# ayushpradhan-dev/robust-speech-analysis-framework

Measured on AMD Instinct MI355X. Metric: audio-seconds processed/sec (extract+CNN-LSTM fwd), higher is better.
Workload: dtype f32

## Files before the change

robust_speech_analysis_framework_amd/csrc/gemm_f16x3.h:

```cpp
#pragma once
#include "gemm_f32.h"

namespace rsaf {

struct GemmH3Params {
    const uint16_t* A;
    int64_t a_plane, lda, sA;
    const float* a_scale;
    int a_scale_zs, a_scale_ms;
    const uint16_t* B;
    int64_t b_plane, ldb;
    const float* b_scale;
    float* C;
    int64_t ldc, sC;
    uint16_t* Cp;
    int64_t c_plane, ldcp, sCp;
    const float* c_scale;
    int c_scale_zs, c_scale_ms;
    unsigned* amax_out;
    int amax_zs;
    const int* amax_row_slot;
    int amax_col_min;
    const float* bias;
    const float* R;
    int64_t ldr, sR;
    int M, N, K, nz;
    const int64_t* ztab;
    const int* row_tab;
    int act;
    float alpha;
    int group_m;
    int a_panel, b_panel, cp_panel;
    int nz2;
    int64_t sA2, sB2, sC2, sBias2;
    int b_panel_rows;
    int a_panel_rows, a_tap_panels, a_tap_inv;
};

int launch_gemm_f16x3(const GemmH3Params& p, hipStream_t stream, const char* tag);

int launch_f16x2_row_scales(const float* src, int64_t rows, int K, int64_t ld, float* scale, float* norm2, unsigned* stat_max,
                            hipStream_t stream);
int launch_split_f16x2(const float* src, int64_t rows, int K, int64_t ld, const float* scale, int scale_stride, uint16_t* planes,
                       int64_t plane_stride, int panels, hipStream_t stream);
int launch_scale_from_bound(const unsigned* amax_bits, int64_t n, const float* factor_dev, float factor_host, const float* add_dev,
                            float* scale, hipStream_t stream);

__host__ __device__ inline float f16x2_scale_for_bound(float bound) {
    union { float f; unsigned u; } v;
    v.f = bound;
    const int e = (int)((v.u >> 23) & 0xff);
    if (e == 0) return 1.0f;
    int se = 127 + 14 - (e - 127);
    se = se < 1 ? 1 : (se > 254 ? 254 : se);
    v.u = (unsigned)se << 23;
    return v.f;
}
__host__ __device__ inline float pow2_inverse(float s) {
    union { float f; unsigned u; } v;
    v.f = s;
    v.u = 0x7F000000u - v.u;
    return v.f;
}

#if defined(__HIPCC__)
typedef float gelu_f32x2 __attribute__((ext_vector_type(2)));
__device__ __forceinline__ gelu_f32x2 gelu_pair(gelu_f32x2 x) {
    const gelu_f32x2 a = x * 0.70710678118654752440f;
    gelu_f32x2 t;
    t.x = __builtin_fabsf(a.x); t.y = __builtin_fabsf(a.y);
    const gelu_f32x2 s = a * a;
    auto K = [](float v) { return gelu_f32x2{v, v}; };
    gelu_f32x2 r = __builtin_elementwise_fma(K(-2.4937484340625815e-05f), t, K(5.528365727514029e-04f));
    const gelu_f32x2 u = __builtin_elementwise_fma(K(-5.603376310318708e-03f), t, K(3.4992024302482605e-02f));
    r = __builtin_elementwise_fma(r, s, u);
    r = __builtin_elementwise_fma(r, t, K(-1.540479063987732e-01f));
    r = __builtin_elementwise_fma(r, t, K(-9.158901572227478e-01f));
    r = __builtin_elementwise_fma(r, t, K(-1.8570011854171753e-01f));
    r = __builtin_elementwise_fma(r, t, t * -1.4426950216293335f);
    gelu_f32x2 e;
    e.x = __builtin_amdgcn_exp2f(r.x); e.y = __builtin_amdgcn_exp2f(r.y);
    gelu_f32x2 far = K(1.0f) - e;
    far.x = __builtin_copysignf(far.x, a.x); far.y = __builtin_copysignf(far.y, a.y);
    gelu_f32x2 q = __builtin_elementwise_fma(K(-5.96761703e-4f), s, K(4.99119423e-3f));
    q = __builtin_elementwise_fma(q, s, K(-2.67681349e-2f));
    q = __builtin_elementwise_fma(q, s, K(1.12819925e-1f));
    q = __builtin_elementwise_fma(q, s, K(-3.76125336e-1f));
    q = __builtin_elementwise_fma(q, s, K(1.28379166e-1f));
    const gelu_f32x2 near = __builtin_elementwise_fma(q, a, a);
    gelu_f32x2 er;
    er.x = t.x > 0.927734375f ? far.x : near.x;
    er.y = t.y > 0.927734375f ? far.y : near.y;
    const gelu_f32x2 hx = x * 0.5f;
    return __builtin_elementwise_fma(hx, er, hx);
}
#endif

}
```

robust_speech_analysis_framework_amd/csrc/gemm_f16x3.hip:

```cpp
#include <algorithm>

#include "gemm_f16x3.h"

namespace rsaf {

using f32x16 = __attribute__((ext_vector_type(16))) float;
using f16x8 = __attribute__((ext_vector_type(8))) _Float16;
typedef __attribute__((address_space(3))) void* lds_ptr3;
typedef const __attribute__((address_space(1))) void* glb_ptr3;

__device__ __forceinline__ unsigned short f16_bits(_Float16 h) { return __builtin_bit_cast(unsigned short, h); }

__device__ __forceinline__ void split2(float xs, unsigned short& h, unsigned short& l) {
    const _Float16 hh = (_Float16)xs;
    const _Float16 ll = (_Float16)(xs - (float)hh);
    h = f16_bits(hh);
    l = f16_bits(ll);
}

template <int TM_, int TN_, int WM_, int WN_, int NST_, int WGS_>
struct H3Cfg {
    static constexpr int TM = TM_, TN = TN_, WM = WM_, WN = WN_, NST = NST_, WGS = WGS_;
    static constexpr int BM = 32 * TM * WM, BN = 32 * TN * WN, BK = 16, NPL = 2;
    static constexpr int THREADS = 64 * WM * WN;
    static constexpr int A_PLANE = BM * BK, B_PLANE = BN * BK;
    static constexpr int STAGE = NPL * (A_PLANE + B_PLANE);
    static constexpr int A_INSTR = BM / 32, B_INSTR = BN / 32;
    static constexpr int PATCH_BYTES = WM * WN * 32 * 36 * 4;
    static constexpr int TAB_BYTES = 2 * (BM + BN) * 4 + 2 * BM * 4;
    static constexpr bool PATCH_IN_STAGE2 = BM > 256;
    static_assert(!PATCH_IN_STAGE2 || STAGE * 2 >= PATCH_BYTES, "stage 2 must hold the epilogue patches");
    static constexpr int LDS_BYTES = NST * STAGE * 2 + (PATCH_IN_STAGE2 ? 0 : PATCH_BYTES) + TAB_BYTES;
};

#if defined(__HIP_DEVICE_COMPILE__)
#define H3_OPAQUE(SP, LB) asm volatile("" : "+s"(SP), "+v"(LB))
#else
#define H3_OPAQUE(SP, LB) (void)0
#endif
#define H3_ADDR(UNIFORM_BASE, LANE_BYTES)                                                                      \
    ({                                                                                                         \
        const char* sp_ = reinterpret_cast<const char*>(UNIFORM_BASE);                                         \
        unsigned lb_ = (LANE_BYTES);                                                                           \
        H3_OPAQUE(sp_, lb_);                                                                                   \
        (glb_ptr3)(sp_ + lb_);                                                                                 \
    })

template <class CFG, int ACT, bool OUT_F32, bool OUT_PLANES, bool HAS_R, bool ROWTAB = false>
__global__ __launch_bounds__(CFG::THREADS, CFG::WGS * CFG::THREADS / 256) void gemm_f16x3_kernel(const GemmH3Params p) {
    extern __shared__ __attribute__((aligned(1024))) unsigned short smem3[];
    constexpr int BM = CFG::BM, BN = CFG::BN, BK = CFG::BK, STAGE = CFG::STAGE, NST = CFG::NST, NPL = CFG::NPL;
    constexpr int TM = CFG::TM, TN = CFG::TN, NW = CFG::WM * CFG::WN;
    constexpr int A_PLANE = CFG::A_PLANE, B_PLANE = CFG::B_PLANE;

    const int tid = threadIdx.x, lane = tid & 63, wave = __builtin_amdgcn_readfirstlane(tid >> 6), l31 = lane & 31, h = lane >> 5;
    const int tiles_n = (p.N + BN - 1) / BN, tiles_m = (p.M + BM - 1) / BM;
    const int nwg = tiles_n * tiles_m;
    const int64_t total_tiles = (int64_t)nwg * p.nz;
    const int wm0 = (wave / CFG::WN) * (32 * TM), wn0 = (wave % CFG::WN) * (32 * TN);

    struct Tile { int m0, n0, Mz; int64_t z, z1, z2, coff; };
    auto tile_at = [&](int64_t t) {
        Tile T;
        T.z = t / nwg;
        const int orig = (int)(t - T.z * nwg);
        T.z1 = p.nz2 > 1 ? T.z / p.nz2 : T.z;
        T.z2 = p.nz2 > 1 ? T.z % p.nz2 : 0;
        T.Mz = p.ztab ? (int)p.ztab[2 * T.z1] : p.M;
        T.coff = p.ztab ? p.ztab[2 * T.z1 + 1] : -1;
        const int xcd = orig & 7, q8 = nwg >> 3, r8 = nwg & 7;
        const int wg = (xcd < r8 ? xcd * (q8 + 1) : r8 * (q8 + 1) + (xcd - r8) * q8) + (orig >> 3);
        const int GROUP_M = p.group_m;
        const int per_group = GROUP_M * tiles_n;
        const int grp = wg / per_group;
        const int first_m = grp * GROUP_M;
        const int gsz = (tiles_m - first_m) < GROUP_M ? (tiles_m - first_m) : GROUP_M;
        const int in_grp = wg - grp * per_group;
        T.m0 = (first_m + in_grp % gsz) * BM;
        T.n0 = (in_grp / gsz) * BN;
        return T;
    };
    auto next_valid = [&](int64_t t, Tile& T) {
        for (; t < total_tiles; t += gridDim.x) {
            T = tile_at(t);
            if (T.m0 < T.Mz) return t;
        }
        return (int64_t)-1;
    };

    constexpr int NI = CFG::A_INSTR + CFG::B_INSTR;
    constexpr int IPW = (NI + NW - 1) / NW;
    const unsigned short* sbase[IPW];
    unsigned voff[IPW];
    int64_t pstride[IPW], kstride[IPW];
    int ldsoff[IPW];
    bool live[IPW];
#pragma unroll
    for (int i = 0; i < IPW; ++i) {
        const int j = wave + NW * i;
        live[i] = j < NI;
        const bool isA = j < CFG::A_INSTR;
        const int jj = isA ? j : j - CFG::A_INSTR;
        pstride[i] = isA ? p.a_plane : p.b_plane;
        kstride[i] = isA ? (p.a_panel ? (int64_t)(p.a_panel_rows > 0 ? p.a_panel_rows : p.M) * 16 : 16) : (p.b_panel ? (int64_t)(p.b_panel_rows > 0 ? p.b_panel_rows : p.N) * 16 : 16);
        ldsoff[i] = isA ? jj * 512 : NPL * A_PLANE + jj * 512;
    }
    auto set_tile = [&](const Tile& T) {
#pragma unroll
        for (int i = 0; i < IPW; ++i) {
            const int j = wave + NW * i;
            const bool isA = j < CFG::A_INSTR;
            const int jj = isA ? j : j - CFG::A_INSTR;
            const int row = 32 * jj + (lane >> 1);
            const int dch = (lane & 1) ^ ((row >> 3) & 1);
            if (isA) {
                const int rr = (T.m0 + row < T.Mz) ? row : T.Mz - 1 - T.m0;
                const int64_t rs = p.a_panel ? 16 : p.lda;
                sbase[i] = p.A + T.z1 * p.sA + T.z2 * p.sA2 + (int64_t)T.m0 * rs;
                voff[i] = 2u * ((unsigned)rr * (unsigned)rs + 8u * dch);
            } else {
                const int rr = (T.n0 + row < p.N) ? row : p.N - 1 - T.n0;
                const int64_t rs = p.b_panel ? 16 : p.ldb;
                sbase[i] = p.B + T.z2 * p.sB2 + (int64_t)T.n0 * rs;
                voff[i] = 2u * ((unsigned)rr * (unsigned)rs + 8u * dch);
            }
        }
    };
    const int nk = p.K / BK;
    auto koff = [&](int i, int KT) -> int64_t {
        if (p.a_tap_panels > 0 && (wave + NW * i) < CFG::A_INSTR) {
            const int tap = (int)(((unsigned)KT * (unsigned)p.a_tap_inv) >> 16);
            return (int64_t)(KT - tap * p.a_tap_panels) * kstride[i] + (int64_t)tap * 16;
        }
        return (int64_t)KT * kstride[i];
    };

#define H3_DMA(KT, ST)                                                                                          \
    do {                                                                                                        \
        _Pragma("unroll") for (int i = 0; i < IPW; ++i) {                                                       \
            if (live[i]) {                                                                                      \
                const bool isA_ = (wave + NW * i) < CFG::A_INSTR;                                               \
                _Pragma("unroll") for (int pl = 0; pl < NPL; ++pl)                                              \
                    __builtin_amdgcn_global_load_lds(H3_ADDR(sbase[i] + (pl * pstride[i] + koff(i, (KT))), voff[i]), \
                        (lds_ptr3)(smem3 + (ST) * STAGE + ldsoff[i] + pl * (isA_ ? A_PLANE : B_PLANE)), 16, 0, 0); \
            }                                                                                                   \
        }                                                                                                       \
    } while (0)

    static_assert(NST == 3 && TM % 2 == 0, "the staggered loop needs three stages and an even number of m-tiles");
    const int grpB = wave >= NW / 2 ? 1 : 0;
    constexpr int NDMA = NPL * IPW;
    constexpr int HM = TM / 2;
    constexpr int PATCH_LD = 36;
    float* patch = reinterpret_cast<float*>(smem3 + (CFG::PATCH_IN_STAGE2 ? 2 : NST) * STAGE) + wave * (32 * PATCH_LD);

    constexpr int TPT = (BM + BN + CFG::THREADS - 1) / CFG::THREADS;
    float* tab0 = reinterpret_cast<float*>(smem3 + NST * STAGE) + (CFG::PATCH_IN_STAGE2 ? 0 : NW * (32 * PATCH_LD));
    float* tab1 = tab0 + (BM + BN);
    int* tab_slot = reinterpret_cast<int*>(tab1 + (BM + BN));
    int* tab_dest = tab_slot + BM;
    float e0[TPT], e1[TPT];
    int e_slot[TPT], e_dest[TPT];
    auto load_epi = [&](const Tile& T) {
#pragma unroll
        for (int u = 0; u < TPT; ++u) {
            const int i = tid + u * CFG::THREADS;
            e0[u] = 1.0f; e1[u] = 0.0f;
            if (i < BM) {
                const int row = T.m0 + i < T.Mz ? T.m0 + i : T.Mz - 1;
                if (ROWTAB) {
                    const int2 rt = reinterpret_cast<const int2*>(p.row_tab)[row];
                    e_slot[u] = rt.x; e_dest[u] = rt.y;
                    e0[u] = p.a_scale[rt.x];
                    e1[u] = (OUT_PLANES && p.Cp) ? p.c_scale[rt.x] : 1.0f;
                } else {
                    e0[u] = p.a_scale[T.z1 * p.a_scale_zs + (int64_t)row * p.a_scale_ms];
                    e1[u] = (OUT_PLANES && p.Cp) ? p.c_scale[T.z1 * p.c_scale_zs + (int64_t)row * p.c_scale_ms] : 1.0f;
                }
            } else if (i < BM + BN) {
                const int col = T.n0 + i - BM;
                e0[u] = col < p.N ? p.b_scale[T.z2 * p.sBias2 + col] : 1.0f;
                e1[u] = (p.bias && col < p.N) ? p.bias[T.z2 * p.sBias2 + col] : 0.0f;
            }
        }
    };
    Tile cur;
    int64_t t_cur = next_valid(blockIdx.x, cur);
    if (t_cur < 0) return;
    load_epi(cur);
    set_tile(cur);
    H3_DMA(0, 0);
    if (nk > 1) H3_DMA(1, 1);

    while (true) {
    f32x16 acc[TM][TN];
#pragma unroll
    for (int i = 0; i < TM; ++i)
#pragma unroll
        for (int j = 0; j < TN; ++j)
#pragma unroll
            for (int e = 0; e < 16; ++e) acc[i][j][e] = 0.0f;

    asm volatile("s_waitcnt vmcnt(0)" ::: "memory");
    if (grpB) __builtin_amdgcn_s_barrier();
    int st = 0;
    for (int kt = 0; kt < nk; ++kt) {
        if (!grpB) asm volatile("s_waitcnt vmcnt(0)" ::: "memory");
        __builtin_amdgcn_s_barrier();
        asm volatile("" ::: "memory");
        const int rkt = kt + 1 + grpB;
        const bool refill = rkt < nk && (grpB || kt >= 1);
        const int rst = (st + 1 + grpB) % NST;
        const unsigned short* img = smem3 + st * STAGE;
        f16x8 bf[TN][NPL];
#pragma unroll
        for (int nt = 0; nt < TN; ++nt) {
            const int row = wn0 + nt * 32 + l31;
            const int off = row * BK + ((h ^ ((row >> 3) & 1)) << 3);
#pragma unroll
            for (int pl = 0; pl < NPL; ++pl) bf[nt][pl] = *reinterpret_cast<const f16x8*>(&img[NPL * A_PLANE + pl * B_PLANE + off]);
        }
        if (refill) {
#pragma unroll
            for (int d = 0; d < NDMA; ++d) {
                const int i = d / NPL, pl = d % NPL;
                if (live[i]) {
                    const bool isA_ = (wave + NW * i) < CFG::A_INSTR;
                    __builtin_amdgcn_sched_barrier(0);
                    __builtin_amdgcn_global_load_lds(H3_ADDR(sbase[i] + (pl * pstride[i] + koff(i, rkt)), voff[i]),
                        (lds_ptr3)(smem3 + rst * STAGE + ldsoff[i] + pl * (isA_ ? A_PLANE : B_PLANE)), 16, 0, 0);
                    __builtin_amdgcn_sched_barrier(0);
                }
            }
        }
        f16x8 afp[NPL];
#pragma unroll
        for (int mt = 0; mt < TM; ++mt) {
            f16x8 af[NPL];
            if (mt == HM) {
#pragma unroll
                for (int pl = 0; pl < NPL; ++pl) af[pl] = afp[pl];
            } else {
                const int row = wm0 + mt * 32 + l31;
                const int off = row * BK + ((h ^ ((row >> 3) & 1)) << 3);
#pragma unroll
                for (int pl = 0; pl < NPL; ++pl) af[pl] = *reinterpret_cast<const f16x8*>(&img[pl * A_PLANE + off]);
            }
            if (mt == HM - 1) {
                const int row = wm0 + HM * 32 + l31;
                const int off = row * BK + ((h ^ ((row >> 3) & 1)) << 3);
#pragma unroll
                for (int pl = 0; pl < NPL; ++pl) afp[pl] = *reinterpret_cast<const f16x8*>(&img[pl * A_PLANE + off]);
            }
#pragma unroll
            for (int nt = 0; nt < TN; ++nt) {
                f32x16 c = acc[mt][nt];
                c = __builtin_amdgcn_mfma_f32_32x32x16_f16(af[1], bf[nt][0], c, 0, 0, 0);
                c = __builtin_amdgcn_mfma_f32_32x32x16_f16(af[0], bf[nt][1], c, 0, 0, 0);
                c = __builtin_amdgcn_mfma_f32_32x32x16_f16(af[0], bf[nt][0], c, 0, 0, 0);
                acc[mt][nt] = c;
            }
            if (mt == HM - 1) {
                if (grpB) {
                    if (!refill) asm volatile("s_waitcnt vmcnt(0)" ::: "memory");
                    else if (live[IPW - 1]) asm volatile("s_waitcnt vmcnt(%0)" ::"n"(NPL * IPW) : "memory");
                    else asm volatile("s_waitcnt vmcnt(%0)" ::"n"(NPL * (IPW - 1) > 0 ? NPL * (IPW - 1) : 0) : "memory");
                }
                __builtin_amdgcn_s_barrier();
                asm volatile("" ::: "memory");
            }
        }
        st = st == NST - 1 ? 0 : st + 1;
    }
    if (!grpB) __builtin_amdgcn_s_barrier();

    const Tile done = cur;
    constexpr int CW = (OUT_PLANES && !OUT_F32) ? 8 : 4, LPR = 32 / CW, RPI = 64 / LPR, NQ = 32 / RPI;
    const int lr = lane / LPR, c4 = CW * (lane % LPR);
    float4 r4[4];
    auto load_r = [&](int mt, int nt) {
        const int tn = done.n0 + wn0 + nt * 32, tm = done.m0 + wm0 + mt * 32;
        const float* Rt = p.R + done.z * p.sR + (int64_t)tm * p.ldr + tn + c4;
#pragma unroll
        for (int q = 0; q < 4; ++q) {
            const bool ok = (tn + c4) < p.N && (tm + 8 * q + lr) < done.Mz;
            r4[q] = (ok && p.R) ? *reinterpret_cast<const float4*>(Rt + (8 * q + lr) * (int)p.ldr) : make_float4(0.f, 0.f, 0.f, 0.f);
        }
    };
#pragma unroll
    for (int u = 0; u < TPT; ++u) {
        const int i = tid + u * CFG::THREADS;
        if (i < BM + BN) { tab0[i] = e0[u]; tab1[i] = e1[u]; }
        if (ROWTAB && i < BM) { tab_slot[i] = e_slot[u]; tab_dest[i] = e_dest[u]; }
    }
    if (HAS_R) load_r(0, 0);

    __syncthreads();
    t_cur = next_valid(t_cur + gridDim.x, cur);
    if (t_cur >= 0) {
        set_tile(cur);
        load_epi(cur);
        H3_DMA(0, 0);
        if (nk > 1) H3_DMA(1, 1);
    }

    {
    const int m0 = done.m0, n0 = done.n0, Mz = done.Mz;
    const int64_t z = done.z, z1 = done.z1, z2 = done.z2;
    static_assert(!HAS_R || CW == 4, "the residual comes with the fp32 output");
#pragma unroll
    for (int mt = 0; mt < TM; ++mt) {
        const int tm = m0 + wm0 + mt * 32;
        float asi[NQ], csc[NQ], row_amax[NQ];
        int drow[NQ];
#pragma unroll
        for (int q = 0; q < NQ; ++q) {
            asi[q] = p.alpha * pow2_inverse(tab0[wm0 + mt * 32 + RPI * q + lr]);
            csc[q] = tab1[wm0 + mt * 32 + RPI * q + lr];
            row_amax[q] = 0.0f;
            drow[q] = ROWTAB ? tab_dest[wm0 + mt * 32 + RPI * q + lr] : tm + RPI * q + lr;
        }
#pragma unroll
        for (int nt = 0; nt < TN; ++nt) {
            const int tn = n0 + wn0 + nt * 32;
            const int gc = tn + c4;
            const bool c_ok = gc < p.N;
            float bsi[CW], bias4[CW];
#pragma unroll
            for (int j4 = 0; j4 < CW / 4; ++j4) {
                const float4 bs4 = *reinterpret_cast<const float4*>(tab0 + BM + wn0 + nt * 32 + c4 + 4 * j4);
                const float4 bi4 = *reinterpret_cast<const float4*>(tab1 + BM + wn0 + nt * 32 + c4 + 4 * j4);
                bsi[4 * j4] = pow2_inverse(bs4.x); bsi[4 * j4 + 1] = pow2_inverse(bs4.y);
                bsi[4 * j4 + 2] = pow2_inverse(bs4.z); bsi[4 * j4 + 3] = pow2_inverse(bs4.w);
                bias4[4 * j4] = bi4.x; bias4[4 * j4 + 1] = bi4.y; bias4[4 * j4 + 2] = bi4.z; bias4[4 * j4 + 3] = bi4.w;
            }
            constexpr int LAST = TM * TN - 1;
            const int sub = mt * TN + nt;
#pragma unroll
            for (int e = 0; e < 16; ++e) patch[(4 * h + (e & 3) + 8 * (e >> 2)) * PATCH_LD + l31] = acc[mt][nt][e];
            __builtin_amdgcn_fence(__ATOMIC_RELEASE, "wavefront");
            __builtin_amdgcn_wave_barrier();
            __builtin_amdgcn_fence(__ATOMIC_ACQUIRE, "wavefront");
            float v[NQ][CW];
#pragma unroll
            for (int q = 0; q < NQ; ++q)
#pragma unroll
                for (int j4 = 0; j4 < CW / 4; ++j4) {
                    const float4 t4 = *reinterpret_cast<const float4*>(patch + (RPI * q + lr) * PATCH_LD + c4 + 4 * j4);
                    v[q][4 * j4] = t4.x; v[q][4 * j4 + 1] = t4.y; v[q][4 * j4 + 2] = t4.z; v[q][4 * j4 + 3] = t4.w;
                }
            __builtin_amdgcn_wave_barrier();
#pragma unroll
            for (int q = 0; q < NQ; ++q) {
                float rv[4] = {0.f, 0.f, 0.f, 0.f};
                if (HAS_R) { rv[0] = r4[q % 4].x; rv[1] = r4[q % 4].y; rv[2] = r4[q % 4].z; rv[3] = r4[q % 4].w; }
#pragma unroll
                for (int j = 0; j < CW; ++j) {
                    float y = v[q][j] * (asi[q] * bsi[j]) + bias4[j];
                    if (HAS_R) y += rv[j % 4];
                    if (ACT == ACT_SILU) y = y / (1.0f + expf(-y));
                    v[q][j] = y;
                    if (ACT == ACT_GELU && (j & 1)) {
                        const gelu_f32x2 g2 = gelu_pair(gelu_f32x2{v[q][j - 1], v[q][j]});
                        v[q][j - 1] = g2.x; v[q][j] = g2.y;
                    }
                    if (ACT != ACT_NONE && (j & 3) == 3) __builtin_amdgcn_sched_barrier(0);
                }
            }
            if (HAS_R && sub < LAST) load_r((sub + 1) / TN, (sub + 1) % TN);
#pragma unroll
            for (int q = 0; q < NQ; ++q) {
                const int row = drow[q];
                const bool ok = c_ok && tm + RPI * q + lr < Mz && (!ROWTAB || row >= 0);
                if (p.amax_out && ok && gc >= p.amax_col_min) {
#pragma unroll
                    for (int j = 0; j < CW; ++j) row_amax[q] = fmaxf(row_amax[q], fabsf(v[q][j]));
                }
                if (ok) {
                    if (OUT_F32 && p.C) *reinterpret_cast<float4*>(p.C + (done.coff >= 0 ? done.coff : z1 * p.sC) + z2 * p.sC2 + (int64_t)row * p.ldc + gc) =
                        make_float4(v[q][0], v[q][1], v[q][2], v[q][3]);
                    if (OUT_PLANES && p.Cp) {
                        const float cs = csc[q];
                        unsigned short hh[CW], ll[CW];
#pragma unroll
                        for (int j = 0; j < CW; ++j) split2(v[q][j] * cs, hh[j], ll[j]);
                        unsigned short* Pt = p.cp_panel ? p.Cp + (int64_t)(gc >> 4) * ((int64_t)p.M * 16) + (int64_t)row * 16 + (gc & 15)
                                                        : p.Cp + z * p.sCp + (int64_t)row * p.ldcp + gc;
                        if (CW == 8) {
                            *reinterpret_cast<uint4*>(Pt) = make_uint4(hh[0] | ((unsigned)hh[1] << 16), hh[2] | ((unsigned)hh[3] << 16),
                                                                      hh[4 % CW] | ((unsigned)hh[5 % CW] << 16), hh[6 % CW] | ((unsigned)hh[7 % CW] << 16));
                            *reinterpret_cast<uint4*>(Pt + p.c_plane) = make_uint4(ll[0] | ((unsigned)ll[1] << 16), ll[2] | ((unsigned)ll[3] << 16),
                                                                                  ll[4 % CW] | ((unsigned)ll[5 % CW] << 16), ll[6 % CW] | ((unsigned)ll[7 % CW] << 16));
                        } else {
                            *reinterpret_cast<uint2*>(Pt) = make_uint2(hh[0] | ((unsigned)hh[1] << 16), hh[2] | ((unsigned)hh[3] << 16));
                            *reinterpret_cast<uint2*>(Pt + p.c_plane) = make_uint2(ll[0] | ((unsigned)ll[1] << 16), ll[2] | ((unsigned)ll[3] << 16));
                        }
                    }
                }
            }
        }
        if (p.amax_out) {
#pragma unroll
            for (int q = 0; q < NQ; ++q) {
                const int row = tm + RPI * q + lr;
                const bool r_ok = row < Mz && (!ROWTAB || drow[q] >= 0);
                const int slot = !r_ok ? -1 : ROWTAB ? tab_slot[wm0 + mt * 32 + RPI * q + lr]
                                                     : (int)(z1 * p.amax_zs) + (p.amax_row_slot ? p.amax_row_slot[row] : 0);
                unsigned long long todo = __ballot(r_ok);
                while (todo) {
                    const int first = __ffsll((long long)todo) - 1;
                    const int s0 = __shfl(slot, first, 64);
                    const bool mine = r_ok && slot == s0;
                    float mx = mine ? row_amax[q] : 0.0f;
#pragma unroll
                    for (int o = 32; o >= 1; o >>= 1) mx = fmaxf(mx, __shfl_xor(mx, o, 64));
                    if (lane == first && mx > 0.0f) atomicMax(p.amax_out + s0, __float_as_uint(mx));
                    todo &= ~__ballot(mine);
                }
            }
        }
    }
    }
    if (t_cur < 0) break;
    }
#undef H3_DMA
}

__global__ __launch_bounds__(256) void f16x2_row_scales_kernel(const float* __restrict__ src, int64_t rows, int K, int64_t ld,
                                                               float* __restrict__ scale, float* __restrict__ norm2,
                                                               unsigned* __restrict__ stat_max) {
    const int64_t row = (int64_t)blockIdx.x * 4 + (threadIdx.x >> 6);
    if (row >= rows) return;
    const int lane = threadIdx.x & 63;
    const float* x = src + row * ld;
    float mx = 0.0f;
    double ss = 0.0;
    for (int k = lane; k < K; k += 64) {
        const float v = x[k];
        mx = fmaxf(mx, fabsf(v));
        ss += (double)v * (double)v;
    }
#pragma unroll
    for (int o = 32; o >= 1; o >>= 1) mx = fmaxf(mx, __shfl_xor(mx, o, 64));
    ss = wave_sum_f64(ss);
    if (lane == 0) {
        scale[row] = f16x2_scale_for_bound(mx);
        const float nn = (float)sqrt(ss) * 1.0000002f;
        if (norm2) norm2[row] = nn;
        if (stat_max) {
            atomicMax(stat_max + 0, __float_as_uint(nn));
            atomicMax(stat_max + 1, __float_as_uint(mx));
        }
    }
}

__global__ __launch_bounds__(256) void split_f16x2_kernel(const float* __restrict__ src, int64_t rows, int K, int64_t ld,
                                                          const float* __restrict__ scale, int scale_stride,
                                                          unsigned short* __restrict__ planes, int64_t plane_stride, int panels) {
    const int64_t row = (int64_t)blockIdx.x * 256 + threadIdx.x;
    if (row >= rows) return;
    const int kb = blockIdx.y;
    const float s = scale[row * scale_stride];
    const float4* s4 = reinterpret_cast<const float4*>(src + row * ld + 16 * kb);
    unsigned short h[16], l[16];
#pragma unroll
    for (int q = 0; q < 4; ++q) {
        const float4 v = s4[q];
        split2(v.x * s, h[4 * q], l[4 * q]); split2(v.y * s, h[4 * q + 1], l[4 * q + 1]);
        split2(v.z * s, h[4 * q + 2], l[4 * q + 2]); split2(v.w * s, h[4 * q + 3], l[4 * q + 3]);
    }
    auto pk = [](const unsigned short* s_, int o) {
        return make_uint4(s_[o] | ((unsigned)s_[o + 1] << 16), s_[o + 2] | ((unsigned)s_[o + 3] << 16),
                          s_[o + 4] | ((unsigned)s_[o + 5] << 16), s_[o + 6] | ((unsigned)s_[o + 7] << 16));
    };
    unsigned short* d = panels ? planes + (int64_t)kb * rows * 16 + row * 16 : planes + row * K + 16 * kb;
    *reinterpret_cast<uint4*>(d) = pk(h, 0); *reinterpret_cast<uint4*>(d + 8) = pk(h, 8);
    *reinterpret_cast<uint4*>(d + plane_stride) = pk(l, 0); *reinterpret_cast<uint4*>(d + plane_stride + 8) = pk(l, 8);
}

__global__ __launch_bounds__(256) void scale_from_bound_kernel(const unsigned* __restrict__ amax_bits, int64_t n,
                                                               const float* __restrict__ factor_dev, float factor_host,
                                                               const float* __restrict__ add_dev, float* __restrict__ scale) {
    const int64_t i = (int64_t)blockIdx.x * 256 + threadIdx.x;
    if (i >= n) return;
    const float f = factor_host * (factor_dev ? *factor_dev : 1.0f);
    const float a = add_dev ? *add_dev : 0.0f;
    scale[i] = f16x2_scale_for_bound(__uint_as_float(amax_bits[i]) * f + a);
}

int launch_f16x2_row_scales(const float* src, int64_t rows, int K, int64_t ld, float* scale, float* norm2, unsigned* stat_max,
                            hipStream_t stream) {
    RSAF_CHECK_ARG(rows >= 0 && K >= 0 && ld >= K, "bad shape");
    if (rows == 0) return RSAF_OK;
    RSAF_CHECK_ARG(src && scale, "NULL pointer");
    RSAF_CHECK_ARG((rows + 3) / 4 <= 0x7fffffffLL, "too many rows");
    hipLaunchKernelGGL(f16x2_row_scales_kernel, dim3((unsigned)((rows + 3) / 4)), dim3(256), 0, stream, src, rows, K, ld, scale, norm2,
                       stat_max);
    RSAF_CHECK_HIP(hipGetLastError());
    return RSAF_OK;
}

int launch_split_f16x2(const float* src, int64_t rows, int K, int64_t ld, const float* scale, int scale_stride, uint16_t* planes,
                       int64_t plane_stride, int panels, hipStream_t stream) {
    RSAF_CHECK_ARG(rows >= 0 && K >= 0 && K % 16 == 0 && ld % 4 == 0 && ld >= K, "K must be a non-negative multiple of 16, ld a multiple of 4");
    if (rows == 0 || K == 0) return RSAF_OK;
    RSAF_CHECK_ARG(src && planes && scale, "NULL pointer");
    RSAF_CHECK_ARG(plane_stride % 8 == 0 && K / 16 <= 65535 && (scale_stride == 0 || scale_stride == 1),
                   "plane stride must be a multiple of 8 elements; at most 65535 panels; scale stride 0 or 1");
    RSAF_CHECK_ARG((reinterpret_cast<uintptr_t>(src) & 15) == 0 && (reinterpret_cast<uintptr_t>(planes) & 15) == 0, "16-byte alignment");
    ProfScope prof("split_f16x2", stream, 0.0, 8.0 * (double)rows * K);
    hipLaunchKernelGGL(split_f16x2_kernel, dim3((unsigned)((rows + 255) / 256), (unsigned)(K / 16)), dim3(256), 0, stream, src, rows, K,
                       ld, scale, scale_stride, reinterpret_cast<unsigned short*>(planes), plane_stride, panels);
    RSAF_CHECK_HIP(hipGetLastError());
    return RSAF_OK;
}

int launch_scale_from_bound(const unsigned* amax_bits, int64_t n, const float* factor_dev, float factor_host, const float* add_dev,
                            float* scale, hipStream_t stream) {
    if (n <= 0) return RSAF_OK;
    RSAF_CHECK_ARG(amax_bits && scale, "NULL pointer");
    hipLaunchKernelGGL(scale_from_bound_kernel, dim3((unsigned)((n + 255) / 256)), dim3(256), 0, stream, amax_bits, n, factor_dev,
                       factor_host, add_dev, scale);
    RSAF_CHECK_HIP(hipGetLastError());
    return RSAF_OK;
}

int launch_gemm_f16x3(const GemmH3Params& p, hipStream_t stream, const char* tag) {
    RSAF_CHECK_ARG(p.M >= 0 && p.N >= 0 && p.K >= 0 && p.nz >= 0, "negative dimension");
    if (p.M == 0 || p.N == 0 || p.nz == 0) return RSAF_OK;
    RSAF_CHECK_ARG(p.A && p.B && (p.C || p.Cp), "NULL operand");
    RSAF_CHECK_ARG(p.a_scale && p.b_scale && (!p.Cp || p.c_scale), "every plane operand needs its scales");
    RSAF_CHECK_ARG(p.K % 16 == 0 && p.K >= 16, "K must be a positive multiple of 16");
    RSAF_CHECK_ARG(p.N % 16 == 0, "N must be a multiple of 16 (16-byte epilogue stores)");
    RSAF_CHECK_ARG(p.ldc % 8 == 0 && p.ldcp % 8 == 0 && p.ldr % 4 == 0 && p.c_plane % 8 == 0 && p.sC % 4 == 0 && p.sCp % 8 == 0 &&
                   p.sR % 4 == 0 && p.sC2 % 4 == 0, "ldc / ldr / output strides must keep 16-byte alignment");
    RSAF_CHECK_ARG(p.lda % 8 == 0 && p.ldb % 8 == 0 && p.a_plane % 8 == 0 && p.b_plane % 8 == 0 && p.sA % 8 == 0 && p.sA2 % 8 == 0 &&
                   p.sB2 % 8 == 0, "lda, ldb, the plane strides and the batch strides must be multiples of 8 elements");
    RSAF_CHECK_ARG((reinterpret_cast<uintptr_t>(p.A) & 15) == 0 && (reinterpret_cast<uintptr_t>(p.B) & 15) == 0 &&
                   (reinterpret_cast<uintptr_t>(p.b_scale) & 15) == 0 && p.sBias2 % 4 == 0, "A, B and b_scale must be 16-byte aligned");
    RSAF_CHECK_ARG(!p.R || p.ldr > 0, "residual needs ldr");
    RSAF_CHECK_ARG(p.act >= 0 && p.act <= 2, "act must be 0 (none), 1 (gelu) or 2 (silu)");
    RSAF_CHECK_ARG(p.nz <= 65535, "at most 65535 batches per launch");
    RSAF_CHECK_ARG(!p.cp_panel || p.nz == 1, "the panel layout of the plane output is for unbatched operands");
    RSAF_CHECK_ARG(!p.a_panel || p.nz == 1 || p.a_panel_rows > 0, "a batched A in panels needs a_panel_rows");
    RSAF_CHECK_ARG(p.a_tap_panels == 0 || (p.a_panel && p.a_panel_rows > 0 && p.a_tap_panels > 0 && (p.K / 16) % p.a_tap_panels == 0),
                   "a_tap_panels: A in panels with a_panel_rows, K = taps x a_tap_panels x 16");
    RSAF_CHECK_ARG(p.ldc < (1 << 24) && p.ldcp < (1 << 24) && p.ldr < (1 << 24), "leading dimensions must be below 2^24");
    RSAF_CHECK_ARG(!p.R || p.C, "the residual comes with the fp32 output");
    RSAF_CHECK_ARG(!p.row_tab || (p.nz == 1 && !p.ztab && p.nz2 <= 1 && !p.cp_panel && !p.a_panel && !p.amax_row_slot),
                   "a row table: one batch, row-major A and plane output, no ztab / amax_row_slot");
    RSAF_CHECK_ARG(p.nz2 <= 1 || (p.C && !p.Cp && !p.R && (!p.a_panel || p.a_panel_rows > 0) && p.nz % p.nz2 == 0),
                   "two-level batches: fp32 output only, no residual, A row-major or panels with a_panel_rows, nz a multiple of nz2");
    ProfScope prof(tag ? tag : "gemm_f16x3", stream, 2.0 * p.M * (double)p.N * p.K * p.nz, 0.0);
    using CfgA = H3Cfg<4, 2, 2, 4, 3, 1>;
    using CfgN = H3Cfg<2, 1, 4, 2, 3, 1>;
    using CfgM = H3Cfg<4, 2, 4, 2, 3, 1>;
#define H3_LAUNCH_CFG(CFG, ACT, F32, PL, HR, ...)                                                                       \
    do {                                                                                                                \
        RSAF_CHECK_HIP(hipFuncSetAttribute((const void*)gemm_f16x3_kernel<CFG, ACT, F32, PL, HR, ##__VA_ARGS__>,         \
                                           hipFuncAttributeMaxDynamicSharedMemorySize, CFG::LDS_BYTES));                 \
        const int64_t tiles = (int64_t)((p.N + CFG::BN - 1) / CFG::BN) * ((p.M + CFG::BM - 1) / CFG::BM) * p.nz;        \
        RSAF_CHECK_ARG(tiles <= 0x7fffffffLL, "too many tiles");                                                        \
        hipLaunchKernelGGL((gemm_f16x3_kernel<CFG, ACT, F32, PL, HR, ##__VA_ARGS__>),                                    \
                           dim3((unsigned)std::min<int64_t>(tiles, persistent_wgs)), dim3(CFG::THREADS), CFG::LDS_BYTES, stream, pp); \
    } while (0)
#define H3_LAUNCH(ACT, F32, PL, HR, ...)                                                                                \
    do {                                                                                                                \
        if (p.N <= 64) H3_LAUNCH_CFG(CfgN, ACT, F32, PL, HR, ##__VA_ARGS__);                                             \
        else H3_LAUNCH_CFG(CfgA, ACT, F32, PL, HR, ##__VA_ARGS__);                                                       \
    } while (0)
#define H3_LAUNCH3(ACT, F32, PL, HR)                                                                                    \
    do {                                                                                                                \
        if (p.N <= 64) H3_LAUNCH_CFG(CfgN, ACT, F32, PL, HR);                                                            \
        else if (p.N <= 128) H3_LAUNCH_CFG(CfgM, ACT, F32, PL, HR);                                                      \
        else H3_LAUNCH_CFG(CfgA, ACT, F32, PL, HR);                                                                      \
    } while (0)
    GemmH3Params pp = p;
    if (pp.group_m <= 0) pp.group_m = 2;
    if (pp.a_tap_panels > 0) {
        pp.a_tap_inv = 65536 / pp.a_tap_panels + 1;
        for (int kt = 0; kt < pp.K / 16; ++kt)
            RSAF_CHECK_ARG((int)(((unsigned)kt * (unsigned)pp.a_tap_inv) >> 16) == kt / pp.a_tap_panels, "a_tap_panels: K too long for the reciprocal");
    }
    int persistent_wgs = 256;
    {
        int dev = 0, cus = 0;
        if (hipGetDevice(&dev) == hipSuccess && hipDeviceGetAttribute(&cus, hipDeviceAttributeMultiprocessorCount, dev) == hipSuccess && cus > 0)
            persistent_wgs = cus;
    }
    const bool f32o = p.C != nullptr, plo = p.Cp != nullptr, hr = p.R != nullptr;
    if (p.row_tab) {
        if (p.act == ACT_GELU && !f32o && plo && !hr) H3_LAUNCH(ACT_GELU, false, true, false, true);
        else if (p.act == ACT_GELU && f32o && !plo && !hr) H3_LAUNCH(ACT_GELU, true, false, false, true);
        else {
            set_error("launch_gemm_f16x3: a row table comes with GELU and one output (planes or fp32)");
            return RSAF_ERR_ARG;
        }
    } else if (p.act == ACT_NONE && f32o && !plo && !hr) H3_LAUNCH3(ACT_NONE, true, false, false);
    else if (p.act == ACT_NONE && f32o && !plo && hr) H3_LAUNCH(ACT_NONE, true, false, true);
    else if (p.act == ACT_GELU && !f32o && plo && !hr) H3_LAUNCH3(ACT_GELU, false, true, false);
    else if (p.act == ACT_SILU && !f32o && plo && !hr) H3_LAUNCH3(ACT_SILU, false, true, false);
    else if (p.act == ACT_GELU && f32o && !plo && !hr) H3_LAUNCH(ACT_GELU, true, false, false);
    else if (p.act == ACT_SILU && f32o && !plo && !hr) H3_LAUNCH(ACT_SILU, true, false, false);
    else if (p.act == ACT_GELU && f32o && !plo && hr) H3_LAUNCH3(ACT_GELU, true, false, true);
    else if (p.act == ACT_SILU && f32o && !plo && hr) H3_LAUNCH3(ACT_SILU, true, false, true);
    else if (p.act == ACT_NONE && !f32o && plo && !hr) H3_LAUNCH(ACT_NONE, false, true, false);
    else if (p.act == ACT_NONE && f32o && plo && !hr) H3_LAUNCH(ACT_NONE, true, true, false);
    else {
        set_error("launch_gemm_f16x3: unsupported combination of activation / outputs / residual");
        return RSAF_ERR_ARG;
    }
#undef H3_LAUNCH_CFG
#undef H3_LAUNCH
#undef H3_LAUNCH3
    RSAF_CHECK_HIP(hipGetLastError());
    return RSAF_OK;
}

}

using namespace rsaf;

extern "C" int rsaf_f16x2_row_scales(const float* src, int64_t rows, int K, int64_t ld, float* scale, float* norm2,
                                     rsaf_stream_t stream) {
    return launch_f16x2_row_scales(src, rows, K, ld, scale, norm2, nullptr, (hipStream_t)stream);
}

extern "C" int rsaf_split_f16x2(const float* src, int64_t rows, int K, int64_t ld, const float* scale, int scale_stride,
                                uint16_t* planes, int64_t plane_stride, int panels, rsaf_stream_t stream) {
    return launch_split_f16x2(src, rows, K, ld, scale, scale_stride, planes, plane_stride, panels, (hipStream_t)stream);
}

extern "C" int rsaf_gemm_f16x3(const uint16_t* A_planes, int64_t a_plane_stride, const float* a_scale, int a_scale_stride,
                               const uint16_t* B_planes, int64_t b_plane_stride, const float* b_scale, float* C,
                               uint16_t* C_planes, int64_t c_plane_stride, const float* c_scale, int c_scale_stride,
                               uint32_t* amax_out, const float* bias, const float* R, int M, int N, int K, int64_t lda, int64_t ldb,
                               int64_t ldc, int64_t ldr, int act, float alpha, int a_panels, int b_panels, int c_panels,
                               rsaf_stream_t stream) {
    GemmH3Params p{};
    p.A = A_planes; p.a_plane = a_plane_stride; p.lda = a_panels ? 16 : lda; p.sA = 0;
    p.a_scale = a_scale; p.a_scale_zs = 0; p.a_scale_ms = a_scale_stride;
    p.B = B_planes; p.b_plane = b_plane_stride; p.ldb = b_panels ? 16 : ldb; p.b_scale = b_scale;
    p.C = C; p.ldc = ldc; p.sC = 0;
    p.Cp = C_planes; p.c_plane = c_plane_stride; p.ldcp = c_panels ? 16 : ldc; p.sCp = 0;
    p.c_scale = c_scale; p.c_scale_zs = 0; p.c_scale_ms = c_scale_stride;
    p.amax_out = amax_out; p.amax_zs = 0; p.amax_row_slot = nullptr; p.amax_col_min = 0;
    p.bias = bias; p.R = R; p.ldr = ldr; p.sR = 0;
    p.M = M; p.N = N; p.K = K; p.nz = 1; p.act = act; p.alpha = alpha;
    p.a_panel = a_panels != 0; p.b_panel = b_panels != 0; p.cp_panel = c_panels != 0;
    return launch_gemm_f16x3(p, (hipStream_t)stream, "gemm_f16x3");
}
```

Measured before the change: 11580.

## Precompute tile-index divisors and advance DMA source pointers incrementally in f16x3 GEMM

Moves per-tile index math to host-precomputed magic-number divisions and tile counts in the params, and replaces per-k-step offset recomputation (tap reciprocal, per-slot strides) with per-plane source pointers advanced by a fixed step or wrap jump. The k-loop is split into compile-time specialised refill and no-refill variants per wave group, removing runtime branches and sched barriers around the DMA issue. The next tile is looked up before the main loop. This cuts scalar and vector address arithmetic in the inner loop, at the cost of more live pointer registers and host-side divisor validation.

```diff
diff --git a/robust_speech_analysis_framework_amd/csrc/gemm_f16x3.h b/robust_speech_analysis_framework_amd/csrc/gemm_f16x3.h
--- a/robust_speech_analysis_framework_amd/csrc/gemm_f16x3.h
+++ b/robust_speech_analysis_framework_amd/csrc/gemm_f16x3.h
@@ -1,7 +1,33 @@
 #pragma once
+#if defined(__HIPCC__)
 #include "gemm_f32.h"
+#define H3_HD __host__ __device__ inline
+#else
+#include <cstdint>
+#define H3_HD inline
+#endif
 
 namespace rsaf {
+
+struct H3Div { unsigned mul; int shift; };
+inline H3Div h3_div_make(int d) {
+    int l = 0;
+    while ((1LL << l) < d) ++l;
+    const uint64_t two = 1ULL << (31 + l);
+    H3Div r;
+    r.mul = (unsigned)((two + (uint64_t)d - 1) / (uint64_t)d);
+    r.shift = 31 + l;
+    return r;
+}
+H3_HD int h3_div(int n, H3Div r) { return (int)(((uint64_t)(unsigned)n * r.mul) >> r.shift); }
+inline bool h3_div_check(H3Div r, int d, int nmax) {
+    if (d <= 0 || nmax < 0 || (uint64_t)r.mul * (uint64_t)d < (1ULL << r.shift)) return false;
+    const int64_t top = (int64_t)(nmax / d) * d;
+    const int64_t at[] = {0, 1, d - 1, d, (int64_t)d + 1, 2LL * d - 1, top - 1, top, top + d - 1, nmax - 1, nmax};
+    for (int64_t n : at)
+        if (n >= 0 && n <= nmax && h3_div((int)n, r) != (int)(n / d)) return false;
+    return true;
+}
 
 struct GemmH3Params {
     const uint16_t* A;
@@ -35,8 +61,57 @@
     int64_t sA2, sB2, sC2, sBias2;
     int b_panel_rows;
     int a_panel_rows, a_tap_panels, a_tap_inv;
+    int tiles_m, tiles_n, nwg;
+    H3Div inv_nwg, inv_nz2, inv_per_group, inv_gsz, inv_gsz_last;
 };
 
+struct H3Tile { int z, z1, z2, tm, tn; };
+H3_HD H3Tile h3_tile_at(const GemmH3Params& p, int t) {
+    H3Tile T;
+    T.z = h3_div(t, p.inv_nwg);
+    const int orig = t - T.z * p.nwg;
+    T.z1 = h3_div(T.z, p.inv_nz2);
+    T.z2 = T.z - T.z1 * (p.nz2 > 1 ? p.nz2 : 1);
+    const int xcd = orig & 7, q8 = p.nwg >> 3, r8 = p.nwg & 7;
+    const int wg = (xcd < r8 ? xcd * (q8 + 1) : r8 * (q8 + 1) + (xcd - r8) * q8) + (orig >> 3);
+    const int per_group = p.group_m * p.tiles_n;
+    const int grp = h3_div(wg, p.inv_per_group);
+    const int first_m = grp * p.group_m;
+    const bool full = p.tiles_m - first_m >= p.group_m;
+    const int gsz = full ? p.group_m : p.tiles_m - first_m;
+    const int in_grp = wg - grp * per_group;
+    T.tn = h3_div(in_grp, full ? p.inv_gsz : p.inv_gsz_last);
+    T.tm = first_m + (in_grp - T.tn * gsz);
+    return T;
+}
+inline bool h3_grid_fill(GemmH3Params& p, int bm, int bn) {
+    const int64_t tn = (p.N + bn - 1) / bn, tm = (p.M + bm - 1) / bm;
+    if (tn <= 0 || tm <= 0 || p.nz <= 0 || p.group_m <= 0 || tn * tm * p.nz > 0x7fffffffLL || p.group_m * tn > 0x7fffffffLL) return false;
+    p.tiles_m = (int)tm; p.tiles_n = (int)tn; p.nwg = (int)(tm * tn);
+    const int nz2 = p.nz2 > 1 ? p.nz2 : 1, per_group = (int)(p.group_m * tn);
+    const int last = p.tiles_m % p.group_m ? p.tiles_m % p.group_m : p.group_m;
+    p.inv_nwg = h3_div_make(p.nwg); p.inv_nz2 = h3_div_make(nz2); p.inv_per_group = h3_div_make(per_group);
+    p.inv_gsz = h3_div_make(p.group_m); p.inv_gsz_last = h3_div_make(last);
+    return h3_div_check(p.inv_nwg, p.nwg, (int)(tm * tn * p.nz - 1)) && h3_div_check(p.inv_nz2, nz2, p.nz - 1) &&
+           h3_div_check(p.inv_per_group, per_group, p.nwg - 1) && h3_div_check(p.inv_gsz, p.group_m, per_group - 1) &&
+           h3_div_check(p.inv_gsz_last, last, per_group - 1);
+}
+
+struct H3KStep { int64_t step, jump; int wrap; };
+H3_HD H3KStep h3_kstep(int64_t kstride, int tap_panels, int unit) {
+    H3KStep s;
+    s.step = kstride * unit;
+    s.jump = tap_panels > 0 ? (16 - (int64_t)(tap_panels - 1) * kstride) * unit : s.step;
+    s.wrap = tap_panels > 0 ? tap_panels : 0x7fffffff;
+    return s;
+}
+H3_HD int64_t h3_kstep_next(const H3KStep& s, int& pc) {
+    const bool w = pc + 1 == s.wrap;
+    pc = w ? 0 : pc + 1;
+    return w ? s.jump : s.step;
+}
+
+#if defined(__HIPCC__)
 int launch_gemm_f16x3(const GemmH3Params& p, hipStream_t stream, const char* tag);
 
 int launch_f16x2_row_scales(const float* src, int64_t rows, int K, int64_t ld, float* scale, float* norm2, unsigned* stat_max,
@@ -46,7 +121,7 @@
 int launch_scale_from_bound(const unsigned* amax_bits, int64_t n, const float* factor_dev, float factor_host, const float* add_dev,
                             float* scale, hipStream_t stream);
 
-__host__ __device__ inline float f16x2_scale_for_bound(float bound) {
+H3_HD float f16x2_scale_for_bound(float bound) {
     union { float f; unsigned u; } v;
     v.f = bound;
     const int e = (int)((v.u >> 23) & 0xff);
@@ -56,14 +131,13 @@
     v.u = (unsigned)se << 23;
     return v.f;
 }
-__host__ __device__ inline float pow2_inverse(float s) {
+H3_HD float pow2_inverse(float s) {
     union { float f; unsigned u; } v;
     v.f = s;
     v.u = 0x7F000000u - v.u;
     return v.f;
 }
 
-#if defined(__HIPCC__)
 typedef float gelu_f32x2 __attribute__((ext_vector_type(2)));
 __device__ __forceinline__ gelu_f32x2 gelu_pair(gelu_f32x2 x) {
     const gelu_f32x2 a = x * 0.70710678118654752440f;
diff --git a/robust_speech_analysis_framework_amd/csrc/gemm_f16x3.hip b/robust_speech_analysis_framework_amd/csrc/gemm_f16x3.hip
--- a/robust_speech_analysis_framework_amd/csrc/gemm_f16x3.hip
+++ b/robust_speech_analysis_framework_amd/csrc/gemm_f16x3.hip
@@ -1,4 +1,5 @@
 #include <algorithm>
+#include <type_traits>
 
 #include "gemm_f16x3.h"
 
@@ -54,102 +55,95 @@
     constexpr int A_PLANE = CFG::A_PLANE, B_PLANE = CFG::B_PLANE;
 
     const int tid = threadIdx.x, lane = tid & 63, wave = __builtin_amdgcn_readfirstlane(tid >> 6), l31 = lane & 31, h = lane >> 5;
-    const int tiles_n = (p.N + BN - 1) / BN, tiles_m = (p.M + BM - 1) / BM;
-    const int nwg = tiles_n * tiles_m;
-    const int64_t total_tiles = (int64_t)nwg * p.nz;
+    const unsigned total_tiles = (unsigned)p.nwg * (unsigned)p.nz;
     const int wm0 = (wave / CFG::WN) * (32 * TM), wn0 = (wave % CFG::WN) * (32 * TN);
 
-    struct Tile { int m0, n0, Mz; int64_t z, z1, z2, coff; };
-    auto tile_at = [&](int64_t t) {
+    struct Tile { int m0, n0, Mz, z, z1, z2; int64_t coff, aoff, boff; unsigned t; bool valid; };
+    auto next_valid = [&](unsigned t) {
         Tile T;
-        T.z = t / nwg;
-        const int orig = (int)(t - T.z * nwg);
-        T.z1 = p.nz2 > 1 ? T.z / p.nz2 : T.z;
-        T.z2 = p.nz2 > 1 ? T.z % p.nz2 : 0;
-        T.Mz = p.ztab ? (int)p.ztab[2 * T.z1] : p.M;
-        T.coff = p.ztab ? p.ztab[2 * T.z1 + 1] : -1;
-        const int xcd = orig & 7, q8 = nwg >> 3, r8 = nwg & 7;
-        const int wg = (xcd < r8 ? xcd * (q8 + 1) : r8 * (q8 + 1) + (xcd - r8) * q8) + (orig >> 3);
-        const int GROUP_M = p.group_m;
-        const int per_group = GROUP_M * tiles_n;
-        const int grp = wg / per_group;
-        const int first_m = grp * GROUP_M;
-        const int gsz = (tiles_m - first_m) < GROUP_M ? (tiles_m - first_m) : GROUP_M;
-        const int in_grp = wg - grp * per_group;
-        T.m0 = (first_m + in_grp % gsz) * BM;
-        T.n0 = (in_grp / gsz) * BN;
+        T.valid = false;
+        for (; t < total_tiles; t += gridDim.x) {
+            const H3Tile W = h3_tile_at(p, (int)t);
+            T.m0 = W.tm * BM; T.n0 = W.tn * BN; T.z = W.z; T.z1 = W.z1; T.z2 = W.z2;
+            T.Mz = p.ztab ? (int)p.ztab[2 * W.z1] : p.M;
+            if (T.m0 < T.Mz) {
+                T.coff = p.ztab ? p.ztab[2 * W.z1 + 1] : -1;
+                T.aoff = W.z1 * p.sA + W.z2 * p.sA2 + (int64_t)T.m0 * (p.a_panel ? 16 : p.lda);
+                T.boff = W.z2 * p.sB2 + (int64_t)T.n0 * (p.b_panel ? 16 : p.ldb);
+                T.t = t; T.valid = true;
+                break;
+            }
+        }
         return T;
     };
-    auto next_valid = [&](int64_t t, Tile& T) {
-        for (; t < total_tiles; t += gridDim.x) {
-            T = tile_at(t);
-            if (T.m0 < T.Mz) return t;
-        }
-        return (int64_t)-1;
-    };
 
     constexpr int NI = CFG::A_INSTR + CFG::B_INSTR;
     constexpr int IPW = (NI + NW - 1) / NW;
-    const unsigned short* sbase[IPW];
+    constexpr int A_SLOTS = CFG::A_INSTR / NW;
+    constexpr int LAST_LIVE = NI - NW * (IPW - 1);
+    static_assert(CFG::A_INSTR % NW == 0, "a slot is an A or a B instruction for every wave alike");
+    static_assert(LAST_LIVE == NW || LAST_LIVE <= NW / 2, "the waves of group B have the same number of DMA instructions");
+    const bool last_live = LAST_LIVE == NW || wave < LAST_LIVE;
+#define H3_LIVE(i) ((i) < IPW - 1 || last_live)
+    const char* src[IPW][NPL];
     unsigned voff[IPW];
-    int64_t pstride[IPW], kstride[IPW];
     int ldsoff[IPW];
-    bool live[IPW];
+    int pc = 0;
+    const H3KStep a_step = h3_kstep(p.a_panel ? (int64_t)(p.a_panel_rows > 0 ? p.a_panel_rows : p.M) * 16 : 16, p.a_tap_panels, 2);
+    const int64_t b_step = 2 * (p.b_panel ? (int64_t)(p.b_panel_rows > 0 ? p.b_panel_rows : p.N) * 16 : 16);
 #pragma unroll
     for (int i = 0; i < IPW; ++i) {
-        const int j = wave + NW * i;
-        live[i] = j < NI;
-        const bool isA = j < CFG::A_INSTR;
-        const int jj = isA ? j : j - CFG::A_INSTR;
-        pstride[i] = isA ? p.a_plane : p.b_plane;
-        kstride[i] = isA ? (p.a_panel ? (int64_t)(p.a_panel_rows > 0 ? p.a_panel_rows : p.M) * 16 : 16) : (p.b_panel ? (int64_t)(p.b_panel_rows > 0 ? p.b_panel_rows : p.N) * 16 : 16);
-        ldsoff[i] = isA ? jj * 512 : NPL * A_PLANE + jj * 512;
+        const int jj = i < A_SLOTS ? wave + NW * i : wave + NW * i - CFG::A_INSTR;
+        ldsoff[i] = i < A_SLOTS ? jj * 512 : NPL * A_PLANE + jj * 512;
     }
     auto set_tile = [&](const Tile& T) {
+        pc = 0;
 #pragma unroll
         for (int i = 0; i < IPW; ++i) {
-            const int j = wave + NW * i;
-            const bool isA = j < CFG::A_INSTR;
-            const int jj = isA ? j : j - CFG::A_INSTR;
+            const bool isA = i < A_SLOTS;
+            const int jj = isA ? wave + NW * i : wave + NW * i - CFG::A_INSTR;
             const int row = 32 * jj + (lane >> 1);
             const int dch = (lane & 1) ^ ((row >> 3) & 1);
-            if (isA) {
-                const int rr = (T.m0 + row < T.Mz) ? row : T.Mz - 1 - T.m0;
-                const int64_t rs = p.a_panel ? 16 : p.lda;
-                sbase[i] = p.A + T.z1 * p.sA + T.z2 * p.sA2 + (int64_t)T.m0 * rs;
-                voff[i] = 2u * ((unsigned)rr * (unsigned)rs + 8u * dch);
-            } else {
-                const int rr = (T.n0 + row < p.N) ? row : p.N - 1 - T.n0;
-                const int64_t rs = p.b_panel ? 16 : p.ldb;
-                sbase[i] = p.B + T.z2 * p.sB2 + (int64_t)T.n0 * rs;
-                voff[i] = 2u * ((unsigned)rr * (unsigned)rs + 8u * dch);
-            }
+            const int rr = isA ? ((T.m0 + row < T.Mz) ? row : T.Mz - 1 - T.m0)
+                               : ((T.n0 + row < p.N) ? row : p.N - 1 - T.n0);
+            const int64_t rs = isA ? (p.a_panel ? 16 : p.lda) : (p.b_panel ? 16 : p.ldb);
+            voff[i] = 2u * ((unsigned)rr * (unsigned)rs + 8u * dch);
+            const unsigned short* base = isA ? p.A + T.aoff : p.B + T.boff;
+#pragma unroll
+            for (int pl = 0; pl < NPL; ++pl)
+                src[i][pl] = reinterpret_cast<const char*>(base + pl * (isA ? p.a_plane : p.b_plane));
         }
     };
-    const int nk = p.K / BK;
-    auto koff = [&](int i, int KT) -> int64_t {
-        if (p.a_tap_panels > 0 && (wave + NW * i) < CFG::A_INSTR) {
-            const int tap = (int)(((unsigned)KT * (unsigned)p.a_tap_inv) >> 16);
-            return (int64_t)(KT - tap * p.a_tap_panels) * kstride[i] + (int64_t)tap * 16;
-        }
-        return (int64_t)KT * kstride[i];
-    };
-
-#define H3_DMA(KT, ST)                                                                                          \
+#define H3_DMA(ST)                                                                                              \
     do {                                                                                                        \
         _Pragma("unroll") for (int i = 0; i < IPW; ++i) {                                                       \
-            if (live[i]) {                                                                                      \
-                const bool isA_ = (wave + NW * i) < CFG::A_INSTR;                                               \
+            if (H3_LIVE(i)) {                                                                                   \
                 _Pragma("unroll") for (int pl = 0; pl < NPL; ++pl)                                              \
-                    __builtin_amdgcn_global_load_lds(H3_ADDR(sbase[i] + (pl * pstride[i] + koff(i, (KT))), voff[i]), \
-                        (lds_ptr3)(smem3 + (ST) * STAGE + ldsoff[i] + pl * (isA_ ? A_PLANE : B_PLANE)), 16, 0, 0); \
+                    __builtin_amdgcn_global_load_lds(H3_ADDR(src[i][pl], voff[i]),                              \
+                        (lds_ptr3)(smem3 + (ST) + ldsoff[i] + pl * (i < A_SLOTS ? A_PLANE : B_PLANE)), 16, 0, 0); \
             }                                                                                                   \
         }                                                                                                       \
     } while (0)
+#define H3_ADVANCE()                                                                                            \
+    do {                                                                                                        \
+        const int64_t a_inc_ = h3_kstep_next(a_step, pc);                                                       \
+        _Pragma("unroll") for (int i = 0; i < IPW; ++i)                                                         \
+            _Pragma("unroll") for (int pl = 0; pl < NPL; ++pl) src[i][pl] += i < A_SLOTS ? a_inc_ : b_step;     \
+    } while (0)
+    const int nk = p.K / BK;
+    auto prefetch = [&](const Tile& T) {
+        set_tile(T);
+        H3_DMA(0);
+        if (nk > 1) {
+            H3_ADVANCE();
+            H3_DMA(STAGE);
+            H3_ADVANCE();
+        }
+    };
 
     static_assert(NST == 3 && TM % 2 == 0, "the staggered loop needs three stages and an even number of m-tiles");
     const int grpB = wave >= NW / 2 ? 1 : 0;
-    constexpr int NDMA = NPL * IPW;
+    constexpr int NDMA_B = NPL * (LAST_LIVE == NW ? IPW : IPW - 1);
     constexpr int HM = TM / 2;
     constexpr int PATCH_LD = 36;
     float* patch = reinterpret_cast<float*>(smem3 + (CFG::PATCH_IN_STAGE2 ? 2 : NST) * STAGE) + wave * (32 * PATCH_LD);
@@ -174,8 +168,8 @@
                     e0[u] = p.a_scale[rt.x];
                     e1[u] = (OUT_PLANES && p.Cp) ? p.c_scale[rt.x] : 1.0f;
                 } else {
-                    e0[u] = p.a_scale[T.z1 * p.a_scale_zs + (int64_t)row * p.a_scale_ms];
-                    e1[u] = (OUT_PLANES && p.Cp) ? p.c_scale[T.z1 * p.c_scale_zs + (int64_t)row * p.c_scale_ms] : 1.0f;
+                    e0[u] = p.a_scale[(int64_t)T.z1 * p.a_scale_zs + (int64_t)row * p.a_scale_ms];
+                    e1[u] = (OUT_PLANES && p.Cp) ? p.c_scale[(int64_t)T.z1 * p.c_scale_zs + (int64_t)row * p.c_scale_ms] : 1.0f;
                 }
             } else if (i < BM + BN) {
                 const int col = T.n0 + i - BM;
@@ -184,15 +178,13 @@
             }
         }
     };
-    Tile cur;
-    int64_t t_cur = next_valid(blockIdx.x, cur);
-    if (t_cur < 0) return;
+    Tile cur = next_valid(blockIdx.x);
+    if (!cur.valid) return;
     load_epi(cur);
-    set_tile(cur);
-    H3_DMA(0, 0);
-    if (nk > 1) H3_DMA(1, 1);
+    prefetch(cur);
 
     while (true) {
+    const Tile nxt = next_valid(cur.t + gridDim.x);
     f32x16 acc[TM][TN];
 #pragma unroll
     for (int i = 0; i < TM; ++i)
@@ -201,17 +193,13 @@
 #pragma unroll
             for (int e = 0; e < 16; ++e) acc[i][j][e] = 0.0f;
 
-    asm volatile("s_waitcnt vmcnt(0)" ::: "memory");
-    if (grpB) __builtin_amdgcn_s_barrier();
-    int st = 0;
-    for (int kt = 0; kt < nk; ++kt) {
-        if (!grpB) asm volatile("s_waitcnt vmcnt(0)" ::: "memory");
+    int s0 = 0, s1 = STAGE, s2 = 2 * STAGE;
+    auto ktile = [&](auto refill_c, auto grpb_c) __attribute__((always_inline)) {
+        constexpr bool REFILL = decltype(refill_c)::value, GRPB = decltype(grpb_c)::value;
+        if (!GRPB) asm volatile("s_waitcnt vmcnt(0)" ::: "memory");
         __builtin_amdgcn_s_barrier();
         asm volatile("" ::: "memory");
-        const int rkt = kt + 1 + grpB;
-        const bool refill = rkt < nk && (grpB || kt >= 1);
-        const int rst = (st + 1 + grpB) % NST;
-        const unsigned short* img = smem3 + st * STAGE;
+        const unsigned short* img = smem3 + s0;
         f16x8 bf[TN][NPL];
 #pragma unroll
         for (int nt = 0; nt < TN; ++nt) {
@@ -220,18 +208,9 @@
 #pragma unroll
             for (int pl = 0; pl < NPL; ++pl) bf[nt][pl] = *reinterpret_cast<const f16x8*>(&img[NPL * A_PLANE + pl * B_PLANE + off]);
         }
-        if (refill) {
-#pragma unroll
-            for (int d = 0; d < NDMA; ++d) {
-                const int i = d / NPL, pl = d % NPL;
-                if (live[i]) {
-                    const bool isA_ = (wave + NW * i) < CFG::A_INSTR;
-                    __builtin_amdgcn_sched_barrier(0);
-                    __builtin_amdgcn_global_load_lds(H3_ADDR(sbase[i] + (pl * pstride[i] + koff(i, rkt)), voff[i]),
-                        (lds_ptr3)(smem3 + rst * STAGE + ldsoff[i] + pl * (isA_ ? A_PLANE : B_PLANE)), 16, 0, 0);
-                    __builtin_amdgcn_sched_barrier(0);
-                }
-            }
+        if (REFILL) {
+            H3_DMA(GRPB ? s2 : s1);
+            H3_ADVANCE();
         }
         f16x8 afp[NPL];
 #pragma unroll
@@ -261,18 +240,27 @@
                 acc[mt][nt] = c;
             }
             if (mt == HM - 1) {
-                if (grpB) {
-                    if (!refill) asm volatile("s_waitcnt vmcnt(0)" ::: "memory");
-                    else if (live[IPW - 1]) asm volatile("s_waitcnt vmcnt(%0)" ::"n"(NPL * IPW) : "memory");
-                    else asm volatile("s_waitcnt vmcnt(%0)" ::"n"(NPL * (IPW - 1) > 0 ? NPL * (IPW - 1) : 0) : "memory");
-                }
+                if (GRPB) asm volatile("s_waitcnt vmcnt(%0)" ::"n"(REFILL ? NDMA_B : 0) : "memory");
                 __builtin_amdgcn_s_barrier();
                 asm volatile("" ::: "memory");
             }
         }
-        st = st == NST - 1 ? 0 : st + 1;
-    }
-    if (!grpB) __builtin_amdgcn_s_barrier();
+        const int s_ = s0; s0 = s1; s1 = s2; s2 = s_;
+    };
+    constexpr std::true_type YES{};
+    constexpr std::false_type NO{};
+    asm volatile("s_waitcnt vmcnt(0)" ::: "memory");
+    if (!grpB) {
+        ktile(NO, NO);
+        for (int kt = 1; kt < nk - 1; ++kt) ktile(YES, NO);
+        if (nk > 1) ktile(NO, NO);
+        __builtin_amdgcn_s_barrier();
+    } else {
+        __builtin_amdgcn_s_barrier();
+        for (int kt = 0; kt < nk - 2; ++kt) ktile(YES, YES);
+        if (nk > 1) ktile(NO, YES);
+        ktile(NO, YES);
+    }
 
     const Tile done = cur;
     constexpr int CW = (OUT_PLANES && !OUT_F32) ? 8 : 4, LPR = 32 / CW, RPI = 64 / LPR, NQ = 32 / RPI;
@@ -280,7 +268,7 @@
     float4 r4[4];
     auto load_r = [&](int mt, int nt) {
         const int tn = done.n0 + wn0 + nt * 32, tm = done.m0 + wm0 + mt * 32;
-        const float* Rt = p.R + done.z * p.sR + (int64_t)tm * p.ldr + tn + c4;
+        const float* Rt = p.R + (int64_t)done.z * p.sR + (int64_t)tm * p.ldr + tn + c4;
 #pragma unroll
         for (int q = 0; q < 4; ++q) {
             const bool ok = (tn + c4) < p.N && (tm + 8 * q + lr) < done.Mz;
@@ -296,12 +284,10 @@
     if (HAS_R) load_r(0, 0);
 
     __syncthreads();
-    t_cur = next_valid(t_cur + gridDim.x, cur);
-    if (t_cur >= 0) {
-        set_tile(cur);
+    cur = nxt;
+    if (cur.valid) {
+        prefetch(cur);
         load_epi(cur);
-        H3_DMA(0, 0);
-        if (nk > 1) H3_DMA(1, 1);
     }
 
     {
@@ -421,9 +407,11 @@
         }
     }
     }
-    if (t_cur < 0) break;
+    if (!cur.valid) break;
     }
 #undef H3_DMA
+#undef H3_ADVANCE
+#undef H3_LIVE
 }
 
 __global__ __launch_bounds__(256) void f16x2_row_scales_kernel(const float* __restrict__ src, int64_t rows, int K, int64_t ld,
@@ -559,8 +547,8 @@
     do {                                                                                                                \
         RSAF_CHECK_HIP(hipFuncSetAttribute((const void*)gemm_f16x3_kernel<CFG, ACT, F32, PL, HR, ##__VA_ARGS__>,         \
                                            hipFuncAttributeMaxDynamicSharedMemorySize, CFG::LDS_BYTES));                 \
-        const int64_t tiles = (int64_t)((p.N + CFG::BN - 1) / CFG::BN) * ((p.M + CFG::BM - 1) / CFG::BM) * p.nz;        \
-        RSAF_CHECK_ARG(tiles <= 0x7fffffffLL, "too many tiles");                                                        \
+        RSAF_CHECK_ARG(h3_grid_fill(pp, CFG::BM, CFG::BN), "too many tiles");                                           \
+        const int64_t tiles = (int64_t)pp.nwg * pp.nz;                                                                  \
         hipLaunchKernelGGL((gemm_f16x3_kernel<CFG, ACT, F32, PL, HR, ##__VA_ARGS__>),                                    \
                            dim3((unsigned)std::min<int64_t>(tiles, persistent_wgs)), dim3(CFG::THREADS), CFG::LDS_BYTES, stream, pp); \
     } while (0)
@@ -577,11 +565,6 @@
     } while (0)
     GemmH3Params pp = p;
     if (pp.group_m <= 0) pp.group_m = 2;
-    if (pp.a_tap_panels > 0) {
-        pp.a_tap_inv = 65536 / pp.a_tap_panels + 1;
-        for (int kt = 0; kt < pp.K / 16; ++kt)
-            RSAF_CHECK_ARG((int)(((unsigned)kt * (unsigned)pp.a_tap_inv) >> 16) == kt / pp.a_tap_panels, "a_tap_panels: K too long for the reciprocal");
-    }
     int persistent_wgs = 256;
     {
         int dev = 0, cus = 0;
```

Measured after the change: 12570 (median of 6 runs). +8.5%, better.
